# zjzijielu/graphsage-simple

Measured on AMD Instinct MI355X. Metric: node-embeddings/sec (2-hop forward), higher is better.
Workload: dtype f32

## Files before the change

### experiments/l2_placement_trace.py

```python
import collections
import csv
import glob
import sys

import numpy as np

f = sorted(glob.glob(sys.argv[1] + "/**/*_kernel_trace.csv", recursive=True))[-1]
edge = int(sys.argv[2]) if len(sys.argv) > 2 else 40


def kind(n):
    if "sample_kernel" in n:
        return "So" if "true, true>" in n else "Si"
    if "layer1_phase_kernel" in n:
        return "G"
    if "layer_tile16" in n or "layer_fused" in n:
        return "L"
    return None


rows = []
for r in csv.DictReader(open(f)):
    k = kind(r["Kernel_Name"])
    if k:
        rows.append((int(r["Start_Timestamp"]), int(r["End_Timestamp"]), k, r.get("Queue_Id", "?")))
rows.sort()
phases = [[rows[0]]]
last = rows[0][1]
for r in rows[1:]:
    if r[0] - last > 300_000:
        phases.append([])
    phases[-1].append(r)
    last = max(last, r[1])
cands = [ph for ph in phases if 100 * 4 <= len(ph) <= 1000 * 4]
big = [ph for ph in phases if len(ph) >= 100 * 4]
p = cands[-1] if cands else big[-1] if big else max(phases, key=len)
print("phases (kernels): " + " ".join(str(len(ph)) for ph in phases if len(ph) >= 50))
by = collections.defaultdict(list)
queues = collections.defaultdict(collections.Counter)
for s, e, k, q in p:
    by[k].append((s, e))
    queues[k][q] += 1
n = min(220, min(len(v) for v in by.values()))
S = {k: np.array(v[-n:], dtype=np.float64) / 1e3 for k, v in by.items()}
assert all((S["L"][:, 0] > S["G"][:, 0]).tolist()) and all((S["G"][:, 0] > S["Si"][:, 0]).tolist()), "kernel kinds do not line up by batch"
lo, hi = edge, n - edge


def stat(x):
    x = np.asarray(x)
    return "avg %5.1f med %5.1f p10 %5.1f p90 %5.1f" % (x.mean(), np.median(x), np.percentile(x, 10), np.percentile(x, 90))


print(f"analysed phase: {n} batches, statistics over batches {lo} .. {hi - 1}")
print("period %.2f us" % ((S["L"][hi - 1, 1] - S["L"][lo, 1]) / (hi - 1 - lo)))
for k in ("So", "Si", "G", "L"):
    print(f"  {k:2s} duration            {stat(S[k][lo:hi, 1] - S[k][lo:hi, 0])}")
print(f"  L(b) start - G(b) end    {stat(S['L'][lo:hi, 0] - S['G'][lo:hi, 1])}")
print(f"  L(b) start - G(b+1) start{stat(S['L'][lo:hi, 0] - S['G'][lo + 1:hi + 1, 0])}")
print(f"  L(b) end - G(b+1) start  {stat(S['L'][lo:hi, 1] - S['G'][lo + 1:hi + 1, 0])}")
print(f"  G(b+1) start - G(b) end  {stat(S['G'][lo + 1:hi + 1, 0] - S['G'][lo:hi, 1])}")
print(f"  G(b) start - Si(b) end   {stat(S['G'][lo:hi, 0] - S['Si'][lo:hi, 1])}")
print(f"  G(b) and G(b+1) together {stat(np.maximum(0.0, S['G'][lo:hi, 1] - S['G'][lo + 1:hi + 1, 0]))}")
print(f"  G end-to-end period      {stat(np.diff(S['G'][lo:hi + 1, 1]))}")
print("  queues used (whole phase): " + "  ".join(f"{k}: " + ", ".join(f"queue {q} x{c}" for q, c in sorted(queues[k].items())) for k in ("So", "Si", "G", "L")))
t0 = S["G"][lo, 0]
print("  timeline of four batches (us from G(b0) start):")
for b in range(lo, lo + 4):
    print("   b=%d " % b + "  ".join(f"{k} {S[k][b, 0] - t0:7.1f}->{S[k][b, 1] - t0:7.1f}" for k in ("So", "Si", "G", "L")))

depth = int(sys.argv[3]) if len(sys.argv) > 3 else 4
ev = sorted((s, e, k, q, i) for k in ("So", "Si", "G", "L") for i, ((s, e), q) in enumerate(zip(by[k][-n:], [r[3] for r in p if r[2] == k][-n:])))
prev_in_queue, last_of_queue = {}, {}
for s, e, k, q, i in ev:
    prev_in_queue[(k, i)] = last_of_queue.get(q)
    last_of_queue[q] = (k, i, e / 1e3)
Q = {(k, i): q for s, e, k, q, i in ev}
producer = {"Si": "So", "G": "Si", "L": "G"}
binding = {k: collections.Counter() for k in ("So", "Si", "G", "L")}
slack = {k: collections.defaultdict(list) for k in ("So", "Si", "G", "L")}
bound_by = {}
for k in ("So", "Si", "G", "L"):
    for b in range(lo, hi):
        start = S[k][b, 0]
        cons = {}
        pq = prev_in_queue[(k, b)]
        if pq:
            cons["queue:%s(b%+d)" % (pq[0], pq[1] - b)] = pq[2]
        if k in producer:
            cons["producer:%s(b)" % producer[k]] = S[producer[k]][b, 1]
        if k == "So" and b - depth >= 0:
            cons["release:L(b-%d)" % depth] = S["L"][b - depth, 1]
        name, t = max(cons.items(), key=lambda kv: kv[1])
        binding[k][name] += 1
        bound_by[(k, b)] = name
        slack[k][name].append(start - t)
print(f"last constraint met before each kernel start (batches {lo} .. {hi - 1}; depth {depth}): count, then start - constraint in us")
# ... 25 lines not shown
```

### graphsage-simple_amd/csrc/sage_api.hip

```cpp
#include <stdarg.h>
#include <string.h>

#include <stdlib.h>

#include <atomic>

#include "sage_internal.h"

static thread_local char g_err[512] = "";

void sage_set_error(const char* fmt, ...) {
    va_list ap;
    va_start(ap, fmt);
    vsnprintf(g_err, sizeof(g_err), fmt, ap);
    va_end(ap);
}

extern "C" int sage_abi_version(void) { return SAGE_ABI_VERSION; }
extern "C" const char* sage_last_error(void) { return g_err; }
extern "C" const char* sage_build_arch(void) { return "gfx950"; }

static int env_int(const char* name, int dflt, int lo, int hi) {
    const char* v = getenv(name);
    if (!v || !*v) return dflt;
    const long x = strtol(v, nullptr, 10);
    return (int)(x < lo ? lo : x > hi ? hi : x);
}

#ifndef SAGE_LAYER1_FUSED_DEFAULT
#define SAGE_LAYER1_FUSED_DEFAULT 1
#endif

const sage_tunables_t& sage_tunables() {
    static const sage_tunables_t t = [] {
        sage_tunables_t x;
        x.gather_blocks_per_cu = env_int("SAGE_G_PER_CU", 6, 1, 8);
        { const int sl = env_int("SAGE_G_SLICE_LANES", 0, 0, 64); x.gather_slice_lanes = (sl == 8 || sl == 16 || sl == 32 || sl == 64) ? sl : 0; }
        x.gather_rows_in_flight = env_int("SAGE_G_ROWS", 1, 1, 4);
        x.gather_trip = env_int("SAGE_G_TRIP", 16, 8, 16) >= 16 ? 16 : 8;
        x.gather_variant = env_int("SAGE_G_VARIANT", 1, 0, 2);
        x.gather_variant_sliced = env_int("SAGE_G_VARIANT_SM", getenv("SAGE_G_VARIANT") ? x.gather_variant : 2, 0, 2);
        x.dense_blocks = env_int("SAGE_DENSE_BLOCKS", 224, 32, 512);
        x.bwd_blocks = env_int("SAGE_BWD_BLOCKS", 512, 16, 4096);
        x.bwd_direct_blocks = env_int("SAGE_BWD_DIRECT_BLOCKS", 256, 16, 1024);
        const int so = env_int("SAGE_SO_THREADS", 512, 256, 1024);
        x.outer_threads = so >= 1024 ? 1024 : so >= 512 ? 512 : 256;
        x.tile16_grid = env_int("SAGE_T16_GRID", 2 * kNumCU, 64, 1024);
        x.sample_fused = env_int("SAGE_SAMPLE_FUSED", 0, 0, 1);
        { const int tw = env_int("SAGE_T16_WAVES", 0, 0, 16); x.tile16_waves = tw == 0 ? 0 : tw >= 16 ? 16 : 8; }
        { const int ti = env_int("SAGE_T16_INFLIGHT", 0, 0, 13); x.tile16_inflight = ti == 0 ? 0 : ti >= 13 ? 13 : 7; }
        x.layer1_fused = env_int("SAGE_LAYER1_FUSED", SAGE_LAYER1_FUSED_DEFAULT, 0, 1);
        x.layer1_phase_per_cu = env_int("SAGE_L1P_PER_CU", 3, 1, 3);
        return x;
    }();
    return t;
}

__global__ void sage_fill_u32_kernel(uint32_t* __restrict__ p, uint32_t v, size_t n_words) {
    for (size_t i = (size_t)blockIdx.x * blockDim.x + threadIdx.x; i < n_words; i += (size_t)gridDim.x * blockDim.x) p[i] = v;
}
int sage_fill_u32(void* p, uint32_t v, size_t n_words, hipStream_t st) {
    if (n_words == 0) return SAGE_OK;
    const int blocks = (int)(n_words < 256 ? 1 : (n_words / 256 < 1024 ? n_words / 256 : 1024));
    hipLaunchKernelGGL(sage_fill_u32_kernel, dim3(blocks), dim3(256), 0, st, (uint32_t*)p, v, n_words);
    SAGE_CHECK_LAUNCH("sage_fill_u32_kernel");
    return SAGE_OK;
}
```

### graphsage-simple_amd/csrc/sage_gather_body.h

```cpp
#pragma once
#include "sage_internal.h"

namespace sage_gather_detail {

template <int SL>
__device__ __forceinline__ void gather_sliced_block(
    const float* __restrict__ table, int table_rows, int64_t ld, int dim,
    const int32_t* __restrict__ nbr, const int32_t* __restrict__ cnt, int k, int n, const int32_t* __restrict__ n_dev,
    const int32_t* __restrict__ slot_rows, const int32_t* __restrict__ self_row, const int32_t* __restrict__ any_nonempty,
    float* __restrict__ out, int64_t ldo, int n_off, int nslice, const int bid, const int nblk, const int64_t slice_stride = 0, const int act = SAGE_ACT_NONE) {
    using V = __attribute__((ext_vector_type(4))) float;
    constexpr int NPI = kWave / SL;
#ifdef SAGE_G_INFLIGHT
    constexpr int U = SAGE_G_INFLIGHT;
#else
    constexpr int U = 8 / NPI;
#endif
    int nn = n;
    if (n_dev) nn = min(*n_dev + n_off, n);
    const int lane = sage_lane();
    const int slice = (int)(bid % nslice);
    const int wave = (int)(((bid / nslice) * blockDim.x + threadIdx.x) >> 6);
    const int nwaves = (int)(((nblk / nslice) * blockDim.x) >> 6);
    const int grp = lane / SL, gl = lane % SL;
// ... 80 lines not shown
            if (self_row) s_cur[i] = self_row[r];
        }
    }
    while (r0 < nn) {
        const int rn0 = r0 + R * nwaves;
        int c_nxt[R], id_nxt[R], s_nxt[R];
#pragma unroll
        for (int i = 0; i < R; ++i) {
            const int r = rn0 + i * nwaves;
            c_nxt[i] = 0; id_nxt[i] = 0; s_nxt[i] = -1;
            if (r < nn) {
                c_nxt[i] = cnt[r];
                id_nxt[i] = (lane < k) ? nbr[(int64_t)r * k + lane] : 0;
                if (self_row) s_nxt[i] = self_row[r];
            }
        }
        int cc[R], ss[R], ids[R];
        bool extra[R];
        V t[R][U];
#pragma unroll
        for (int i = 0; i < R; ++i) {
            cc[i] = min(__builtin_amdgcn_readfirstlane(c_cur[i]), kWave);
            int s = s_cur[i];
            if (slot_rows && s >= 0) s = slot_rows[s];
            ss[i] = __builtin_amdgcn_readfirstlane(s);
            int myid = (lane < cc[i]) ? id_cur[i] : 0;
            if (slot_rows) myid = slot_rows[max(myid, 0)];
            extra[i] = ss[i] >= 0;
            if (extra[i] && __any(lane < cc[i] && myid == ss[i])) extra[i] = false;
            ids[i] = min(max(myid, 0), last_row);
#pragma unroll
            for (int u = 0; u < U; ++u) {
                const int j = u * NPI + grp;
                const int id = __shfl(ids[i], min(j, max(cc[i] - 1, 0)), kWave);
                if (ok && j < cc[i]) t[i][u] = *reinterpret_cast<const V*>(tcol + (int64_t)id * ld);
                else t[i][u] = V{0.f, 0.f, 0.f, 0.f};
            }
        }
#pragma unroll
        for (int i = 0; i < R; ++i) {
            const int r = r0 + i * nwaves;
            if (r >= nn) continue;
            const int c = cc[i];
            V acc = {0.f, 0.f, 0.f, 0.f};
#pragma unroll
            for (int u = 0; u < U; ++u) acc += t[i][u];
            for (int j0 = NPI * U; j0 < c; j0 += NPI * U) {
                V w[U];
#pragma unroll
                for (int u = 0; u < U; ++u) {
                    const int j = j0 + u * NPI + grp;
                    const int id = __shfl(ids[i], min(j, c - 1), kWave);
                    if (ok && j < c) w[u] = *reinterpret_cast<const V*>(tcol + (int64_t)id * ld);
                    else w[u] = V{0.f, 0.f, 0.f, 0.f};
                }
#pragma unroll
                for (int u = 0; u < U; ++u) acc += w[u];
            }
            if (extra[i] && ok && grp == 0) acc += *reinterpret_cast<const V*>(tcol + (int64_t)min(ss[i], last_row) * ld);
#pragma unroll
            for (int m = SL; m < kWave; m <<= 1) {
                acc[0] += __shfl_xor(acc[0], m, kWave);
                acc[1] += __shfl_xor(acc[1], m, kWave);
                acc[2] += __shfl_xor(acc[2], m, kWave);
                acc[3] += __shfl_xor(acc[3], m, kWave);
            }
            if (grp == 0 && ok) {
                const int ceff = c + (extra[i] ? 1 : 0);
                V res;
                if (ceff > 0) res = acc * (1.0f / (float)ceff);
                else { const float fill = nan_rule ? __builtin_nanf("") : 0.f; res = V{fill, fill, fill, fill}; }
                if (act != SAGE_ACT_NONE) { res[0] = sage_activate(res[0], act); res[1] = sage_activate(res[1], act); res[2] = sage_activate(res[2], act); res[3] = sage_activate(res[3], act); }
            sage_store_stream<SAGE_AGG_STORE>(reinterpret_cast<V*>(out + (int64_t)r * ldo + c0), res);
            }
        }
        r0 = rn0;
#pragma unroll
        for (int i = 0; i < R; ++i) { c_cur[i] = c_nxt[i]; id_cur[i] = id_nxt[i]; s_cur[i] = s_nxt[i]; }
    }
}

using gather_v4 = __attribute__((ext_vector_type(4))) float;
template <int TRIP, bool SLOT>
__device__ __forceinline__ gather_v4 gather_rows_unit_sum(const float* __restrict__ tcol, const int64_t ld, const int32_t* __restrict__ myn,
                                                          const int c, const int k, const int s, const int last_row,
                                                          const int32_t* __restrict__ slot_rows, bool& extra) {
    using V = gather_v4;
    V acc = {0.f, 0.f, 0.f, 0.f};
    for (int j0 = 0; j0 < k; j0 += TRIP) {
        int id[TRIP];
#pragma unroll
        for (int u = 0; u < TRIP; ++u) id[u] = myn[min(min(j0 + u, c - 1), k - 1) < 0 ? 0 : min(min(j0 + u, c - 1), k - 1)];
        V t[TRIP];
#pragma unroll
        for (int u = 0; u < TRIP; ++u) {
            int x = id[u];
            if (SLOT) x = slot_rows[max(x, 0)];
            extra = extra && !(j0 + u < c && x == s);
            x = min(max(x, 0), last_row);
            t[u] = *reinterpret_cast<const V*>(tcol + (int64_t)x * ld);
        }
#pragma unroll
        for (int u = 0; u < TRIP; ++u) {
            acc[0] += (j0 + u < c) ? t[u][0] : 0.f; acc[1] += (j0 + u < c) ? t[u][1] : 0.f;
            acc[2] += (j0 + u < c) ? t[u][2] : 0.f; acc[3] += (j0 + u < c) ? t[u][3] : 0.f;
        }
    }
    if (extra) {
        const V sv = *reinterpret_cast<const V*>(tcol + (int64_t)min(s, last_row) * ld);
        acc += sv;
    }
    return acc;
}
__device__ __forceinline__ gather_v4 gather_rows_unit_mean(const gather_v4 acc, const int c, const bool extra, const bool nan_rule) {
    const int ceff = c + (extra ? 1 : 0);
    if (ceff > 0) return acc * (1.0f / (float)ceff);
    const float fill = nan_rule ? __builtin_nanf("") : 0.f;
    return gather_v4{fill, fill, fill, fill};
}

template <int SL, int TRIP, bool SLOT>
__device__ __forceinline__ void gather_sliced_block_rows(
    const float* __restrict__ table, int table_rows, int64_t ld, int dim,
    const int32_t* __restrict__ nbr, const int32_t* __restrict__ cnt, int k, int n, const int32_t* __restrict__ n_dev,
    const int32_t* __restrict__ slot_rows, const int32_t* __restrict__ self_row, const int32_t* __restrict__ any_nonempty,
    float* __restrict__ out, int64_t ldo, int n_off, int nslice, const int bid, const int nblk, const int64_t slice_stride = 0, const int act = SAGE_ACT_NONE) {
    using V = __attribute__((ext_vector_type(4))) float;
    constexpr int NG = kWave / SL;
    int nn = n;
    if (n_dev) nn = min(*n_dev + n_off, n);
    const int lane = sage_lane();
    const int slice = (int)(bid % nslice);
    const int wave = (int)(((bid / nslice) * blockDim.x + threadIdx.x) >> 6);
    const int nwaves = (int)(((nblk / nslice) * blockDim.x) >> 6);
    const int grp = lane / SL, gl = lane % SL;
    const int c0 = min(slice * SL * 4 + gl * 4, dim - 4);
    const bool ok = slice * SL * 4 + gl * 4 < dim;
    const bool nan_rule = any_nonempty ? (*any_nonempty != 0) : false;
    const int last_row = table_rows - 1;
    const float* __restrict__ tcol = table + (slice_stride ? (int64_t)slice * slice_stride + min(gl * 4, SL * 4 - 4) : (int64_t)c0);
    const int nblocks_rows = (nn + NG - 1) / NG;
    for (int rb = wave; rb < nblocks_rows; rb += nwaves) {
        const int r = rb * NG + grp;
        const bool valid = r < nn;
        const int rq = valid ? r : nn - 1;
        const int c = min(cnt[rq], k);
        int s = -1;
        if (self_row) {
            s = self_row[rq];
            if (SLOT && s >= 0) s = slot_rows[s];
        }
        bool extra = s >= 0;
        const int32_t* __restrict__ myn = nbr + (int64_t)rq * k;
        const V acc = gather_rows_unit_sum<TRIP, SLOT>(tcol, ld, myn, c, k, s, last_row, slot_rows, extra);
        if (valid && ok) {
            V res = gather_rows_unit_mean(acc, c, extra, nan_rule);
            if (act != SAGE_ACT_NONE) { res[0] = sage_activate(res[0], act); res[1] = sage_activate(res[1], act); res[2] = sage_activate(res[2], act); res[3] = sage_activate(res[3], act); }
            sage_store_stream<SAGE_AGG_STORE>(reinterpret_cast<V*>(out + (int64_t)r * ldo + c0), res);
        }
    }
}

}
```

### graphsage-simple_amd/csrc/sage_internal.h

```cpp
#pragma once
#include "sage_common.h"

struct sage_resolve_t {
    const int32_t* slots; int32_t* rows_out; int32_t n_slots;
    const int32_t* self_slots; int32_t* self_rows_out; int32_t n_self;
    const int32_t* hash_rows; int32_t* hash_keys;
};
struct sage_slot_resolve_t {
    int32_t* wipe_keys;
    int32_t* rows_out;
    int32_t* self_rows_out;
};
struct sage_finish_t {
    int32_t* counters;
    int32_t* cursor;
};
struct sage_rows_t {
    const float* table; int64_t table_rows; int64_t ld; int32_t dim;
    int64_t slice_stride = 0;
};
struct sage_lists_t {
    const int32_t* nbr = nullptr;
    const int32_t* cnt = nullptr;
    int32_t k = 0;
// ... 35 lines not shown
    const sage_model_t* queue_model = nullptr;
    int nodes_from_batch = 0;
    int32_t* nodes_copy = nullptr;
    const int32_t* seed_map = nullptr;
    const sage_resolve_t* resolve = nullptr;
};
int sage_launch_sample(const sage_sample_t& s, hipStream_t st, sage_launch_events_t* ev = nullptr);
int sage_launch_sample_wide(const sage_sample_t& s, hipStream_t st);
int sage_check_frontier(const sage_frontier_t* f, int64_t inserts);

struct sage_sample_fused_t {
    const sage_model_t* m; const int32_t* seeds; int32_t batch; uint64_t seed; int queued = 0;
    int32_t* nbr2; int32_t* cnt2; int32_t* any2 = nullptr;
    const sage_frontier_t* frontier; int32_t frontier_row_off = 0; int32_t insert_self = 0; int32_t* nbr_slot; int32_t* self_slot = nullptr;
    int32_t* nodes_copy = nullptr;
    int32_t* nbr1; int32_t* cnt1; int32_t* any1 = nullptr; int32_t seed_rows = 0;
};
int sage_launch_sample_fused(const sage_sample_fused_t& s, hipStream_t st);

int sage_launch_gather_mean(const sage_rows_t& src, const sage_lists_t& l, float* out, int64_t ldo, int32_t act, hipStream_t st,
                            sage_launch_events_t* ev = nullptr);
bool sage_layer_dense_supported(int32_t dim, int32_t out_dim);
bool sage_gather_is_sliced(int32_t dim, int64_t ld, int64_t ldo, const float* table, const float* out, int32_t n, int32_t k);

int sage_launch_linear_act(const sage_rows_t& agg, const sage_lists_t& rows, const sage_self_t& self, const sage_contract_t& c,
                           sage_finish_t fin, hipStream_t st);

enum sage_layer_company_t {
    SAGE_BESIDE_ANYTHING = 0,
    SAGE_BESIDE_ONE_WAVE_LAYER1 = 1,
    SAGE_BESIDE_LAYER1_AND_INNER_SAMPLER = 2,
};
int sage_launch_layer_fused(const sage_rows_t& src, const sage_lists_t& l, const sage_self_t& self, const sage_contract_t& c,
                            const sage_slot_resolve_t* resolve, sage_finish_t fin, hipStream_t st, sage_launch_events_t* ev = nullptr,
                            sage_layer_company_t company = SAGE_BESIDE_ANYTHING);
bool sage_layer_fused_supported(int32_t dim, int32_t out_dim, int32_t concat);
int sage_launch_layer_dense(const sage_rows_t& agg, const sage_lists_t& rows, const sage_self_t& self, const sage_contract_t& c,
                            sage_finish_t fin, hipStream_t st, sage_launch_events_t* ev = nullptr);

bool sage_layer1_phase_supported(int32_t d0, int32_t h1, int32_t k);
int sage_launch_layer1_phase(const sage_rows_t& src, const sage_lists_t& l, const sage_contract_t& c, hipStream_t st,
                             sage_launch_events_t* ev = nullptr);

struct sage_head_t {
    const float* emb; int64_t lde; int32_t dim;
    const float* w_cls; int64_t ldw; int32_t num_classes;
    const int64_t* labels = nullptr; int32_t n; float scale = 1.f;
    float* scores = nullptr; int64_t lds = 0; int32_t* pred = nullptr;
    float* grad_emb = nullptr; int64_t ldg = 0;
    float* part_w = nullptr; float* part_loss = nullptr;
    float* grad_w = nullptr; int64_t ldgw = 0; float* loss = nullptr;
};
int sage_launch_xent_head(const sage_head_t& h, hipStream_t st);

#define SAGE_STAGE_SAMPLE_OUTER 1
#define SAGE_STAGE_SAMPLE_INNER 2
#define SAGE_STAGE_GATHER1      4
#define SAGE_STAGE_CONTRACT1    8
#define SAGE_STAGE_LAYER2       16
#define SAGE_STAGE_ALL          31
int sage_forward2_launch_stages(const sage_model_t* m, void* workspace, size_t workspace_bytes, const int32_t* seeds, int32_t batch,
                                uint64_t seed, float* out, int64_t ldo, int32_t stages, hipStream_t stream, void* tail_event = nullptr,
                                void* const* gather_events = nullptr, bool inner_with_layer1 = false);

bool sage_forward2_contract1_is_empty(const sage_model_t* m, int32_t batch);
bool sage_forward2_sampler_is_fused(const sage_model_t* m);

struct sage_tunables_t {
    int gather_blocks_per_cu;
    int gather_slice_lanes;
    int gather_rows_in_flight;
    int gather_trip;
    int gather_variant;
    int gather_variant_sliced;
    int dense_blocks;
    int bwd_blocks;
    int bwd_direct_blocks;
    int outer_threads;
    int tile16_grid;
    int sample_fused;
    int tile16_waves;
    int tile16_inflight;
    int layer1_fused;
    int layer1_phase_per_cu;
};
int sage_fill_u32(void* p, uint32_t v, size_t n_words, hipStream_t st);
const sage_tunables_t& sage_tunables();

#ifndef SAGE_SPLIT_MIN_DIM
#define SAGE_SPLIT_MIN_DIM 64
#endif

#ifdef __HIPCC__
struct sage_finish_regs { int32_t c[7]; int32_t cur; };

__device__ inline void sage_finish_begin(const sage_finish_t& fin, sage_finish_regs& r) {
    if (!fin.counters || threadIdx.x != 0) return;
#pragma unroll
    for (int i = 0; i < 7; ++i) r.c[i] = fin.counters[i];
    r.cur = fin.cursor ? *fin.cursor : 0;
}

__device__ inline void sage_finish_block(const sage_finish_t& fin, int total_blocks, const sage_finish_regs& r) {
    if (!fin.counters) return;
    __syncthreads();
    if (threadIdx.x == 0) {
        if (__hip_atomic_fetch_add(&fin.counters[7], 1, __ATOMIC_RELAXED, __HIP_MEMORY_SCOPE_AGENT) == total_blocks - 1) {
#pragma unroll
            for (int i = 0; i < 7; ++i) {
                fin.counters[8 + i] = r.c[i];
                fin.counters[i] = 0;
            }
            fin.counters[7] = 0;
            if (fin.cursor) *fin.cursor = r.cur + 1;
        }
    }
}

__device__ inline void sage_finish_block(const sage_finish_t& fin, int total_blocks) {
    sage_finish_regs r;
    sage_finish_begin(fin, r);
    sage_finish_block(fin, total_blocks, r);
}
#endif
```

### graphsage-simple_amd/csrc/sage_layer1_phase.hip

```cpp
#include "sage_gather_body.h"
#include "sage_split_bf16.h"

namespace {

using namespace sage_split_detail;
using sage_gather_detail::gather_rows_unit_mean;
using sage_gather_detail::gather_rows_unit_sum;
using sage_gather_detail::gather_v4;

struct PhaseArgs {
    const float* table; int table_rows; int64_t slice_stride;
    const int32_t* nbr; const int32_t* cnt; int k;
    int n; const int32_t* n_dev; int n_off;
    const int32_t* self_row; const int32_t* any_nonempty;
    const float* W; int64_t ldw; const uint4* wsplit; int out_dim; int act;
    float* out; int64_t ldo;
};

constexpr int kTileRows = 32;
constexpr int kSliceFloats = 32;
constexpr int kMaxK = SAGE_MAX_FANOUT;

__device__ inline float exact_mean(const PhaseArgs& a, const int32_t* ids, int c, int s, bool extra, bool nan_rule, int kk) {
    const int last_row = a.table_rows - 1;
    const float* col = a.table + (int64_t)(kk / kSliceFloats) * a.slice_stride + (kk % kSliceFloats);
    float sum = 0.f;
    for (int j = 0; j < c; ++j) sum += col[(int64_t)min(max(ids[j], 0), last_row) * kSliceFloats];
    if (extra) sum += col[(int64_t)min(s, last_row) * kSliceFloats];
    const int ceff = c + (extra ? 1 : 0);
    if (ceff > 0) return sum * (1.0f / (float)ceff);
    return nan_rule ? __builtin_nanf("") : 0.f;
}

template <int NSLICE>
__global__ __launch_bounds__(256, 3) void layer1_phase_kernel(const PhaseArgs a) {
    constexpr int M = kTileRows, SL = 8, TRIP = 16;
    constexpr int LDB = kSliceFloats + 8;
    constexpr int PL = M * LDB;
    constexpr int PLD = 128 + 4;
    constexpr int STEPS = NSLICE;
    __shared__ __attribute__((aligned(16))) __bf16 planes[2 * 3 * PL];
    __shared__ __attribute__((aligned(16))) float outp[M * PLD];
    __shared__ int32_t ids[M * kMaxK];
    __shared__ int32_t cnts[M], selfs[M];
    __shared__ int rowflag[M];
    __shared__ int tileflag;

    const int tid = threadIdx.x, lane = tid & 63, wave = tid >> 6;
    int nn = a.n;
    if (a.n_dev) nn = min(*a.n_dev + a.n_off, a.n);
    const int ntiles = (nn + M - 1) / M;
    const bool nan_rule = a.any_nonempty ? (*a.any_nonempty != 0) : false;
    const int last_row = a.table_rows - 1;
    const int grp = lane / SL, gl = lane % SL;
    const int lr = wave * (kWave / SL) + grp;
    const int i32 = lane & 31, h = lane >> 5;
    const int n0 = wave * 32;
    const bool mfma_wave = n0 < a.out_dim;
    const int k = a.k;
    const bool w_huge = a.wsplit[(size_t)8 * STEPS * 3 * 64].x != 0;

    for (int tile = (int)blockIdx.x; tile < ntiles; tile += (int)gridDim.x) {
        __syncthreads();
        for (int i = tid; i < M * k; i += 256) {
            const int rq = min(tile * M + i / k, nn - 1);
            ids[i] = a.nbr[(int64_t)rq * k + i % k];
        }
        if (tid < M) {
            const int rq = min(tile * M + tid, nn - 1);
            cnts[tid] = min(a.cnt[rq], k);
            selfs[tid] = a.self_row ? a.self_row[rq] : -1;
            rowflag[tid] = 0;
        }
        if (tid == 0) tileflag = w_huge ? 1 : 0;
        __syncthreads();
        const bool valid = tile * M + lr < nn;
        const int c = cnts[lr], s = selfs[lr];
        const int32_t* myn = ids + lr * k;

        f32x16 acc[2];
#pragma unroll
        for (int e = 0; e < 16; ++e) { acc[0][e] = 0.f; acc[1][e] = 0.f; }
#pragma unroll
        for (int kg = 0; kg < 2; ++kg) {
#pragma unroll 1
            for (int q = 0; q < NSLICE / 2; ++q) {
                const int p = kg * (NSLICE / 2) + q;
                const float* tcol = a.table + (int64_t)p * a.slice_stride + gl * 4;
                bool extra = s >= 0;
                const gather_v4 sum = gather_rows_unit_sum<TRIP, false>(tcol, kSliceFloats, myn, c, k, s, last_row, nullptr, extra);
                bf16x8 bw[2][3];
                {
                    const uint4* wp = a.wsplit + ((size_t)(kg * 4 + __builtin_amdgcn_readfirstlane(wave)) * STEPS + 2 * q) * 3 * 64;
#pragma unroll
                    for (int j = 0; j < 2; ++j)
#pragma unroll
                        for (int pl = 0; pl < 3; ++pl) bw[j][pl] = __builtin_bit_cast(bf16x8, wp[(j * 3 + pl) * 64 + lane]);
                }
                gather_v4 res = gather_rows_unit_mean(sum, c, extra, nan_rule);
                if (!valid) res = gather_v4{0.f, 0.f, 0.f, 0.f};
                if (huge4(res)) { rowflag[lr] = 1; tileflag = 1; }
                __bf16* buf = planes + (p & 1) * 3 * PL;
                {
                    bf16x4 hi, mid, lo;
                    split3(res, hi, mid, lo);
                    __bf16* dst = buf + lr * LDB + gl * 4;
                    *reinterpret_cast<bf16x4*>(dst) = hi;
                    *reinterpret_cast<bf16x4*>(dst + PL) = mid;
                    *reinterpret_cast<bf16x4*>(dst + 2 * PL) = lo;
                }
                lds_barrier();
                if (mfma_wave) {
                    const __bf16* abase = buf + i32 * LDB + 8 * h;
#pragma unroll
                    for (int j = 0; j < 2; ++j) {
                        const bf16x8 ah = *reinterpret_cast<const bf16x8*>(abase + 16 * j);
                        const bf16x8 am = *reinterpret_cast<const bf16x8*>(abase + PL + 16 * j);
                        const bf16x8 al = *reinterpret_cast<const bf16x8*>(abase + 2 * PL + 16 * j);
                        acc[kg] = mfma_bf16x3_step(ah, am, al, bw[j], acc[kg]);
                    }
                }
            }
        }
        if (mfma_wave) {
            float* mine = outp + n0 + i32;
#pragma unroll
            for (int reg = 0; reg < 16; ++reg) mine[((reg & 3) + 8 * (reg >> 2) + 4 * h) * PLD] = acc[0][reg] + acc[1][reg];
        }
        lds_barrier();
        const bool any_bad = tileflag != 0;
#pragma unroll
        for (int it = 0; it < M * 32 / 256; ++it) {
            const int idx = it * 256 + tid;
            const int row = idx >> 5, col = (idx & 31) * 4;
            const int g = tile * M + row;
            if (g < nn && col < a.out_dim && !(any_bad && (w_huge || rowflag[row] != 0))) {
                const f32x4 pv = *reinterpret_cast<const f32x4*>(outp + row * PLD + col);
                f32x4 v;
#pragma unroll
                for (int e = 0; e < 4; ++e) v[e] = sage_activate(pv[e], a.act);
                sage_store_stream<SAGE_H1_STORE>(reinterpret_cast<f32x4*>(a.out + (int64_t)g * a.ldo + col), v);
            }
        }
        if (any_bad) {
            const int d0 = NSLICE * kSliceFloats;
            for (int idx = tid; idx < M * a.out_dim; idx += 256) {
                const int row = idx / a.out_dim, col = idx % a.out_dim;
                const int g = tile * M + row;
                if (g >= nn || !(w_huge || rowflag[row] != 0)) continue;
                const int32_t* rid = ids + row * k;
                const int rc = cnts[row], rs = selfs[row];
                bool rextra = rs >= 0;
                for (int j = 0; j < rc; ++j) rextra = rextra && rid[j] != rs;
                const float* wrow = a.W + (int64_t)col * a.ldw;
                float dot = 0.f;
                for (int kk = 0; kk < d0; ++kk) dot = fmaf(exact_mean(a, rid, rc, rs, rextra, nan_rule, kk), wrow[kk], dot);
                a.out[(int64_t)g * a.ldo + col] = sage_activate(dot, a.act);
            }
        }
    }
}

template <int NSLICE>
int launch_phase(const PhaseArgs& a, hipStream_t st, sage_launch_events_t* ev) {
    const int per_cu = sage_tunables().layer1_phase_per_cu;
    const int grid = min((sage_cdiv(a.n, kTileRows) + 7) / 8 * 8, kNumCU * per_cu);
    sage_launch(layer1_phase_kernel<NSLICE>, dim3(grid), dim3(256), 0, st, ev, a);
    SAGE_CHECK_LAUNCH("layer1_phase_kernel");
    return SAGE_OK;
}

}

bool sage_layer1_phase_supported(int32_t d0, int32_t h1, int32_t k) {
    return (d0 == 64 || d0 == 128 || d0 == 256) && h1 >= 32 && h1 <= 128 && h1 % 32 == 0 && k >= 1 && k <= kMaxK;
}

int sage_launch_layer1_phase(const sage_rows_t& src, const sage_lists_t& l, const sage_contract_t& c, hipStream_t st,
                             sage_launch_events_t* ev) {
    const int32_t d0 = src.dim;
    SAGE_REQUIRE(src.ld == kSliceFloats && src.slice_stride == src.table_rows * (int64_t)kSliceFloats,
                 "layer1_fused: the table must be slice-major with %d-float slices", kSliceFloats);
    if (!sage_layer1_phase_supported(d0, c.out_dim, l.k) || !c.weight_prepared || !sage_aligned(src.table, 16) || !sage_aligned(c.out, 16) ||
        !sage_aligned(c.weight_prepared, 16) || c.ldo % 4 != 0 || c.ldo < c.out_dim || c.ldw < d0) {
        sage_set_error("layer1_fused: unsupported shape d0=%d h1=%d k=%d (or unaligned arrays / no prepared weights)", d0, c.out_dim, l.k);
        return SAGE_EUNSUPPORTED;
    }
    if (l.n == 0) return SAGE_OK;
    const PhaseArgs a{src.table, (int)src.table_rows, src.slice_stride, l.nbr, l.cnt, l.k, l.n, l.n_dev, l.n_off, l.self_row, l.any_nonempty,
                      c.weight, c.ldw, (const uint4*)c.weight_prepared, c.out_dim, c.act, c.out, c.ldo};
    if (d0 == 64) return launch_phase<2>(a, st, ev);
    if (d0 == 128) return launch_phase<4>(a, st, ev);
    return launch_phase<8>(a, st, ev);
}

extern "C" int sage_layer1_fused_supported(int32_t d0, int32_t h1, int32_t k) { return sage_layer1_phase_supported(d0, h1, k) ? 1 : 0; }

extern "C" int sage_layer1_fused(const float* table_sliced, int64_t table_rows, int32_t d0, const int32_t* nbr, const int32_t* cnt,
                                 int32_t k, int32_t n, const int32_t* n_dev, const int32_t* self_row, const int32_t* any_nonempty,
                                 const float* weight, int64_t ldw, const void* weight_prepared, int32_t out_dim, int32_t act, float* out,
                                 int64_t ldo, sage_stream_t stream) {
    SAGE_REQUIRE(table_sliced && nbr && cnt && weight && weight_prepared && out, "layer1_fused: NULL array");
    SAGE_REQUIRE(n >= 0 && table_rows >= 1 && table_rows < (1ll << 31), "layer1_fused: n = %d, table_rows = %lld", n, (long long)table_rows);
    SAGE_REQUIRE(act >= 0 && act <= SAGE_ACT_NONE, "layer1_fused: bad activation");
    return sage_launch_layer1_phase({.table = table_sliced, .table_rows = table_rows, .ld = kSliceFloats, .dim = d0,
                                     .slice_stride = table_rows * (int64_t)kSliceFloats},
                                    {.nbr = nbr, .cnt = cnt, .k = k, .n = n, .n_dev = n_dev, .self_row = self_row, .any_nonempty = any_nonempty},
                                    {.weight = weight, .ldw = ldw, .weight_prepared = weight_prepared, .out_dim = out_dim, .act = act, .out = out,
                                     .ldo = ldo},
                                    (hipStream_t)stream);
}
```

Baseline: 80.82 million.

## Add two-tile layer-1 pair kernel that overlaps neighbour gathers with contraction

Adds a layer1_pair_kernel where each block processes two 32-row tiles at once. The neighbour-row gathers for one tile are issued in halves while the other tile's sums and MFMA contraction run, so memory latency is hidden by software pipelining with sched barriers. The kernel is specialised on self-row and long-fanout cases and is the default (SAGE_L1P_TILES=2), with occupancy reduced to 2 blocks per CU. The existing kernel is refactored into shared helpers. The costs are more registers and lower occupancy in exchange for more loads in flight per wave.

```diff
diff --git a/experiments/l2_placement_trace.py b/experiments/l2_placement_trace.py
--- a/experiments/l2_placement_trace.py
+++ b/experiments/l2_placement_trace.py
@@ -12,7 +12,7 @@
 def kind(n):
     if "sample_kernel" in n:
         return "So" if "true, true>" in n else "Si"
-    if "layer1_phase_kernel" in n:
+    if "layer1_phase_kernel" in n or "layer1_pair_kernel" in n:
         return "G"
     if "layer_tile16" in n or "layer_fused" in n:
         return "L"
diff --git a/graphsage-simple_amd/csrc/sage_api.hip b/graphsage-simple_amd/csrc/sage_api.hip
--- a/graphsage-simple_amd/csrc/sage_api.hip
+++ b/graphsage-simple_amd/csrc/sage_api.hip
@@ -31,6 +31,10 @@
 #define SAGE_LAYER1_FUSED_DEFAULT 1
 #endif
 
+#ifndef SAGE_L1P_TILES_DEFAULT
+#define SAGE_L1P_TILES_DEFAULT 2
+#endif
+
 const sage_tunables_t& sage_tunables() {
     static const sage_tunables_t t = [] {
         sage_tunables_t x;
@@ -50,7 +54,8 @@
         { const int tw = env_int("SAGE_T16_WAVES", 0, 0, 16); x.tile16_waves = tw == 0 ? 0 : tw >= 16 ? 16 : 8; }
         { const int ti = env_int("SAGE_T16_INFLIGHT", 0, 0, 13); x.tile16_inflight = ti == 0 ? 0 : ti >= 13 ? 13 : 7; }
         x.layer1_fused = env_int("SAGE_LAYER1_FUSED", SAGE_LAYER1_FUSED_DEFAULT, 0, 1);
-        x.layer1_phase_per_cu = env_int("SAGE_L1P_PER_CU", 3, 1, 3);
+        x.layer1_phase_tiles = env_int("SAGE_L1P_TILES", SAGE_L1P_TILES_DEFAULT, 1, 2);
+        { const int most = x.layer1_phase_tiles == 2 ? 2 : 3; x.layer1_phase_per_cu = env_int("SAGE_L1P_PER_CU", most, 1, most); }
         return x;
     }();
     return t;
diff --git a/graphsage-simple_amd/csrc/sage_gather_body.h b/graphsage-simple_amd/csrc/sage_gather_body.h
--- a/graphsage-simple_amd/csrc/sage_gather_body.h
+++ b/graphsage-simple_amd/csrc/sage_gather_body.h
@@ -186,35 +186,53 @@
 
 using gather_v4 = __attribute__((ext_vector_type(4))) float;
 template <int TRIP, bool SLOT>
+__device__ __forceinline__ void gather_rows_unit_issue(const float* __restrict__ tcol, const int64_t ld, const int32_t* __restrict__ myn,
+                                                       const int j0, const int c, const int k, const int s, const int last_row,
+                                                       const int32_t* __restrict__ slot_rows, bool& extra, gather_v4 (&t)[TRIP]) {
+    int id[TRIP];
+#pragma unroll
+    for (int u = 0; u < TRIP; ++u) id[u] = myn[min(min(j0 + u, c - 1), k - 1) < 0 ? 0 : min(min(j0 + u, c - 1), k - 1)];
+#pragma unroll
+    for (int u = 0; u < TRIP; ++u) {
+        int x = id[u];
+        if (SLOT) x = slot_rows[max(x, 0)];
+        extra = extra && !(j0 + u < c && x == s);
+        x = min(max(x, 0), last_row);
+        t[u] = *reinterpret_cast<const gather_v4*>(tcol + (int64_t)x * ld);
+    }
+}
+template <int TRIP>
+__device__ __forceinline__ void gather_rows_unit_add(gather_v4& acc, const gather_v4 (&t)[TRIP], const int j0, const int c) {
+#pragma unroll
+    for (int u = 0; u < TRIP; ++u) {
+        acc[0] += (j0 + u < c) ? t[u][0] : 0.f; acc[1] += (j0 + u < c) ? t[u][1] : 0.f;
+        acc[2] += (j0 + u < c) ? t[u][2] : 0.f; acc[3] += (j0 + u < c) ? t[u][3] : 0.f;
+    }
+}
+template <int TRIP, bool SLOT>
 __device__ __forceinline__ gather_v4 gather_rows_unit_sum(const float* __restrict__ tcol, const int64_t ld, const int32_t* __restrict__ myn,
                                                           const int c, const int k, const int s, const int last_row,
                                                           const int32_t* __restrict__ slot_rows, bool& extra) {
     using V = gather_v4;
     V acc = {0.f, 0.f, 0.f, 0.f};
     for (int j0 = 0; j0 < k; j0 += TRIP) {
-        int id[TRIP];
-#pragma unroll
-        for (int u = 0; u < TRIP; ++u) id[u] = myn[min(min(j0 + u, c - 1), k - 1) < 0 ? 0 : min(min(j0 + u, c - 1), k - 1)];
         V t[TRIP];
-#pragma unroll
-        for (int u = 0; u < TRIP; ++u) {
-            int x = id[u];
-            if (SLOT) x = slot_rows[max(x, 0)];
-            extra = extra && !(j0 + u < c && x == s);
-            x = min(max(x, 0), last_row);
-            t[u] = *reinterpret_cast<const V*>(tcol + (int64_t)x * ld);
-        }
-#pragma unroll
-        for (int u = 0; u < TRIP; ++u) {
-            acc[0] += (j0 + u < c) ? t[u][0] : 0.f; acc[1] += (j0 + u < c) ? t[u][1] : 0.f;
-            acc[2] += (j0 + u < c) ? t[u][2] : 0.f; acc[3] += (j0 + u < c) ? t[u][3] : 0.f;
-        }
+        gather_rows_unit_issue<TRIP, SLOT>(tcol, ld, myn, j0, c, k, s, last_row, slot_rows, extra, t);
+        gather_rows_unit_add<TRIP>(acc, t, j0, c);
     }
     if (extra) {
         const V sv = *reinterpret_cast<const V*>(tcol + (int64_t)min(s, last_row) * ld);
         acc += sv;
     }
     return acc;
+}
+__device__ __forceinline__ float gather_rows_unit_scale(const int c, const bool extra) {
+    const int ceff = c + (extra ? 1 : 0);
+    return ceff > 0 ? 1.0f / (float)ceff : -1.0f;
+}
+__device__ __forceinline__ gather_v4 gather_rows_unit_mean(const gather_v4 acc, const float scale, const bool nan_rule) {
+    const float fill = nan_rule ? __builtin_nanf("") : 0.f;
+    return scale >= 0.f ? acc * scale : gather_v4{fill, fill, fill, fill};
 }
 __device__ __forceinline__ gather_v4 gather_rows_unit_mean(const gather_v4 acc, const int c, const bool extra, const bool nan_rule) {
     const int ceff = c + (extra ? 1 : 0);
diff --git a/graphsage-simple_amd/csrc/sage_internal.h b/graphsage-simple_amd/csrc/sage_internal.h
--- a/graphsage-simple_amd/csrc/sage_internal.h
+++ b/graphsage-simple_amd/csrc/sage_internal.h
@@ -141,6 +141,7 @@
     int tile16_waves;
     int tile16_inflight;
     int layer1_fused;
+    int layer1_phase_tiles;
     int layer1_phase_per_cu;
 };
 int sage_fill_u32(void* p, uint32_t v, size_t n_words, hipStream_t st);
diff --git a/graphsage-simple_amd/csrc/sage_layer1_phase.hip b/graphsage-simple_amd/csrc/sage_layer1_phase.hip
--- a/graphsage-simple_amd/csrc/sage_layer1_phase.hip
+++ b/graphsage-simple_amd/csrc/sage_layer1_phase.hip
@@ -4,7 +4,10 @@
 namespace {
 
 using namespace sage_split_detail;
+using sage_gather_detail::gather_rows_unit_add;
+using sage_gather_detail::gather_rows_unit_issue;
 using sage_gather_detail::gather_rows_unit_mean;
+using sage_gather_detail::gather_rows_unit_scale;
 using sage_gather_detail::gather_rows_unit_sum;
 using sage_gather_detail::gather_v4;
 
@@ -20,6 +23,9 @@
 constexpr int kTileRows = 32;
 constexpr int kSliceFloats = 32;
 constexpr int kMaxK = SAGE_MAX_FANOUT;
+constexpr int kOutLd = 128 + 4;
+constexpr int kPlaneLd = kSliceFloats + 8;
+constexpr int kPlane = kTileRows * kPlaneLd;
 
 __device__ inline float exact_mean(const PhaseArgs& a, const int32_t* ids, int c, int s, bool extra, bool nan_rule, int kk) {
     const int last_row = a.table_rows - 1;
@@ -32,12 +38,90 @@
     return nan_rule ? __builtin_nanf("") : 0.f;
 }
 
+template <int STEPS>
+__device__ __forceinline__ void load_w1_phase(const uint4* wsplit, const int kg, const int q, const int wave, const int lane, bf16x8 (&bw)[2][3]) {
+    const uint4* wp = wsplit + ((size_t)(kg * 4 + __builtin_amdgcn_readfirstlane(wave)) * STEPS + 2 * q) * 3 * 64;
+#pragma unroll
+    for (int j = 0; j < 2; ++j)
+#pragma unroll
+        for (int pl = 0; pl < 3; ++pl) bw[j][pl] = __builtin_bit_cast(bf16x8, wp[(j * 3 + pl) * 64 + lane]);
+}
+
+__device__ __forceinline__ f32x16 contract_slice(const gather_v4 res, __bf16* buf, const int lr, const int gl, const int lane, const bool mfma_wave,
+                                                 int* rowflag_lr, int* tileflag, const bf16x8 (&bw)[2][3], f32x16 acc) {
+    constexpr int LDB = kPlaneLd, PL = kPlane;
+    if (huge4(res)) { *rowflag_lr = 1; *tileflag = 1; }
+    {
+        bf16x4 hi, mid, lo;
+        split3(res, hi, mid, lo);
+        __bf16* dst = buf + lr * LDB + gl * 4;
+        *reinterpret_cast<bf16x4*>(dst) = hi;
+        *reinterpret_cast<bf16x4*>(dst + PL) = mid;
+        *reinterpret_cast<bf16x4*>(dst + 2 * PL) = lo;
+    }
+    lds_barrier();
+    if (mfma_wave) {
+        const __bf16* abase = buf + (lane & 31) * LDB + 8 * (lane >> 5);
+#pragma unroll
+        for (int j = 0; j < 2; ++j) {
+            const bf16x8 ah = *reinterpret_cast<const bf16x8*>(abase + 16 * j);
+            const bf16x8 am = *reinterpret_cast<const bf16x8*>(abase + PL + 16 * j);
+            const bf16x8 al = *reinterpret_cast<const bf16x8*>(abase + 2 * PL + 16 * j);
+            acc = mfma_bf16x3_step(ah, am, al, bw[j], acc);
+        }
+    }
+    return acc;
+}
+
+template <int NSLICE>
+__device__ __forceinline__ void tile_epilogue(const PhaseArgs& a, const int tile, const int nn, const f32x16 (&acc)[2], float* outp,
+                                              const int32_t* ids, const int32_t* cnts, const int32_t* selfs, const int* rowflag,
+                                              const int* tileflag, const bool w_huge, const bool nan_rule) {
+    constexpr int M = kTileRows, PLD = kOutLd;
+    const int tid = threadIdx.x, lane = tid & 63, wave = tid >> 6;
+    const int i32 = lane & 31, h = lane >> 5, n0 = wave * 32, k = a.k;
+    if (n0 < a.out_dim) {
+        float* mine = outp + n0 + i32;
+#pragma unroll
+        for (int reg = 0; reg < 16; ++reg) mine[((reg & 3) + 8 * (reg >> 2) + 4 * h) * PLD] = acc[0][reg] + acc[1][reg];
+    }
+    lds_barrier();
+    const bool any_bad = *tileflag != 0;
+#pragma unroll 1
+    for (int it = 0; it < M * 32 / 256; ++it) {
+        const int idx = it * 256 + tid;
+        const int row = idx >> 5, col = (idx & 31) * 4;
+        const int g = tile * M + row;
+        if (g < nn && col < a.out_dim && !(any_bad && (w_huge || rowflag[row] != 0))) {
+            const f32x4 pv = *reinterpret_cast<const f32x4*>(outp + row * PLD + col);
+            f32x4 v;
+#pragma unroll
+            for (int e = 0; e < 4; ++e) v[e] = sage_activate(pv[e], a.act);
+            sage_store_stream<SAGE_H1_STORE>(reinterpret_cast<f32x4*>(a.out + (int64_t)g * a.ldo + col), v);
+        }
+    }
+    if (any_bad) {
+        const int d0 = NSLICE * kSliceFloats;
+        for (int idx = tid; idx < M * a.out_dim; idx += 256) {
+            const int row = idx / a.out_dim, col = idx % a.out_dim;
+            const int g = tile * M + row;
+            if (g >= nn || !(w_huge || rowflag[row] != 0)) continue;
+            const int32_t* rid = ids + row * k;
+            const int rc = cnts[row], rs = selfs[row];
+            bool rextra = rs >= 0;
+            for (int j = 0; j < rc; ++j) rextra = rextra && rid[j] != rs;
+            const float* wrow = a.W + (int64_t)col * a.ldw;
+            float dot = 0.f;
+            for (int kk = 0; kk < d0; ++kk) dot = fmaf(exact_mean(a, rid, rc, rs, rextra, nan_rule, kk), wrow[kk], dot);
+            a.out[(int64_t)g * a.ldo + col] = sage_activate(dot, a.act);
+        }
+    }
+}
+
 template <int NSLICE>
 __global__ __launch_bounds__(256, 3) void layer1_phase_kernel(const PhaseArgs a) {
     constexpr int M = kTileRows, SL = 8, TRIP = 16;
-    constexpr int LDB = kSliceFloats + 8;
-    constexpr int PL = M * LDB;
-    constexpr int PLD = 128 + 4;
+    constexpr int PL = kPlane, PLD = kOutLd;
     constexpr int STEPS = NSLICE;
     __shared__ __attribute__((aligned(16))) __bf16 planes[2 * 3 * PL];
     __shared__ __attribute__((aligned(16))) float outp[M * PLD];
@@ -54,9 +138,7 @@
     const int last_row = a.table_rows - 1;
     const int grp = lane / SL, gl = lane % SL;
     const int lr = wave * (kWave / SL) + grp;
-    const int i32 = lane & 31, h = lane >> 5;
-    const int n0 = wave * 32;
-    const bool mfma_wave = n0 < a.out_dim;
+    const bool mfma_wave = wave * 32 < a.out_dim;
     const int k = a.k;
     const bool w_huge = a.wsplit[(size_t)8 * STEPS * 3 * 64].x != 0;
 
@@ -90,80 +172,158 @@
                 bool extra = s >= 0;
                 const gather_v4 sum = gather_rows_unit_sum<TRIP, false>(tcol, kSliceFloats, myn, c, k, s, last_row, nullptr, extra);
                 bf16x8 bw[2][3];
-                {
-                    const uint4* wp = a.wsplit + ((size_t)(kg * 4 + __builtin_amdgcn_readfirstlane(wave)) * STEPS + 2 * q) * 3 * 64;
-#pragma unroll
-                    for (int j = 0; j < 2; ++j)
-#pragma unroll
-                        for (int pl = 0; pl < 3; ++pl) bw[j][pl] = __builtin_bit_cast(bf16x8, wp[(j * 3 + pl) * 64 + lane]);
-                }
+                load_w1_phase<STEPS>(a.wsplit, kg, q, wave, lane, bw);
                 gather_v4 res = gather_rows_unit_mean(sum, c, extra, nan_rule);
                 if (!valid) res = gather_v4{0.f, 0.f, 0.f, 0.f};
-                if (huge4(res)) { rowflag[lr] = 1; tileflag = 1; }
-                __bf16* buf = planes + (p & 1) * 3 * PL;
-                {
-                    bf16x4 hi, mid, lo;
-                    split3(res, hi, mid, lo);
-                    __bf16* dst = buf + lr * LDB + gl * 4;
-                    *reinterpret_cast<bf16x4*>(dst) = hi;
-                    *reinterpret_cast<bf16x4*>(dst + PL) = mid;
-                    *reinterpret_cast<bf16x4*>(dst + 2 * PL) = lo;
-                }
-                lds_barrier();
-                if (mfma_wave) {
-                    const __bf16* abase = buf + i32 * LDB + 8 * h;
-#pragma unroll
-                    for (int j = 0; j < 2; ++j) {
-                        const bf16x8 ah = *reinterpret_cast<const bf16x8*>(abase + 16 * j);
-                        const bf16x8 am = *reinterpret_cast<const bf16x8*>(abase + PL + 16 * j);
-                        const bf16x8 al = *reinterpret_cast<const bf16x8*>(abase + 2 * PL + 16 * j);
-                        acc[kg] = mfma_bf16x3_step(ah, am, al, bw[j], acc[kg]);
-                    }
-                }
+                acc[kg] = contract_slice(res, planes + (p & 1) * 3 * kPlane, lr, gl, lane, mfma_wave, &rowflag[lr], &tileflag, bw, acc[kg]);
             }
         }
-        if (mfma_wave) {
-            float* mine = outp + n0 + i32;
-#pragma unroll
-            for (int reg = 0; reg < 16; ++reg) mine[((reg & 3) + 8 * (reg >> 2) + 4 * h) * PLD] = acc[0][reg] + acc[1][reg];
-        }
+        tile_epilogue<NSLICE>(a, tile, nn, acc, outp, ids, cnts, selfs, rowflag, &tileflag, w_huge, nan_rule);
+    }
+}
+
+template <int NSLICE, bool SELF, bool LONG>
+__global__ __launch_bounds__(256, 2) void layer1_pair_kernel(const PhaseArgs a) {
+    constexpr int M = kTileRows, SL = 8, HALF = 8;
+    constexpr int MORE = 4;
+    constexpr int PL = kPlane, PLD = kOutLd;
+    constexpr int STEPS = NSLICE;
+    __shared__ __attribute__((aligned(16))) __bf16 planes[2 * 3 * PL];
+    __shared__ __attribute__((aligned(16))) float outp[M * PLD];
+    __shared__ int32_t ids[2 * M * kMaxK];
+    __shared__ int32_t cnts[2 * M], selfs[2 * M];
+    __shared__ int rowflag[2 * M];
+    __shared__ int tileflag[2];
+
+    const int tid = threadIdx.x, lane = tid & 63, wave = tid >> 6;
+    int nn = a.n;
+    if (a.n_dev) nn = min(*a.n_dev + a.n_off, a.n);
+    const int npairs = (nn + 2 * M - 1) / (2 * M);
+    const bool nan_rule = a.any_nonempty ? (*a.any_nonempty != 0) : false;
+    const int last_row = a.table_rows - 1;
+    const int grp = lane / SL, gl = lane % SL;
+    const int lr = wave * (kWave / SL) + grp;
+    const bool mfma_wave = wave * 32 < a.out_dim;
+    const int k = a.k;
+    const bool w_huge = a.wsplit[(size_t)8 * STEPS * 3 * 64].x != 0;
+
+    for (int pair = (int)blockIdx.x; pair < npairs; pair += (int)gridDim.x) {
+        __syncthreads();
+        {
+            const int row = tid >> 2;
+            const int rq = min(pair * 2 * M + row, nn - 1);
+            for (int j = tid & 3; j < k; j += 4) ids[row * k + j] = a.nbr[(int64_t)rq * k + j];
+        }
+        if (tid < 2 * M) {
+            const int rq = min(pair * 2 * M + tid, nn - 1);
+            cnts[tid] = min(a.cnt[rq], k);
+            selfs[tid] = SELF ? a.self_row[rq] : -1;
+            rowflag[tid] = 0;
+        }
+        if (tid < 2) tileflag[tid] = w_huge ? 1 : 0;
+        __syncthreads();
+        bool valid[2], extra[2];
+        float scale[2];
+        int c[2], s[2];
+        const int32_t* myn[2];
+#pragma unroll
+        for (int t = 0; t < 2; ++t) {
+            valid[t] = pair * 2 * M + t * M + lr < nn;
+            c[t] = cnts[t * M + lr];
+            s[t] = selfs[t * M + lr];
+            myn[t] = ids + (t * M + lr) * k;
+            extra[t] = SELF && s[t] >= 0;
+            if (SELF)
+                for (int j = 0; j < c[t]; ++j) extra[t] = extra[t] && myn[t][j] != s[t];
+            scale[t] = gather_rows_unit_scale(c[t], extra[t]);
+        }
+        auto issue = [&](const int t, const int p, const int h, gather_v4 (&rows)[HALF], gather_v4& selfv) __attribute__((always_inline)) {
+            const float* tcol = a.table + (int64_t)p * a.slice_stride + gl * 4;
+            bool unused = false;
+            const int cnow = cnts[t * M + lr];
+            gather_rows_unit_issue<HALF, false>(tcol, kSliceFloats, myn[t], HALF * h, cnow, k, -1, last_row, nullptr, unused, rows);
+            if (SELF && h == 0) selfv = *reinterpret_cast<const gather_v4*>(tcol + (int64_t)min(max(selfs[t * M + lr], 0), last_row) * kSliceFloats);
+        };
+        auto finish = [&](const int t, const int p, gather_v4 sum, const gather_v4 selfv) __attribute__((always_inline)) {
+            const float* tcol = a.table + (int64_t)p * a.slice_stride + gl * 4;
+            const int cnow = cnts[t * M + lr];
+            for (int j0 = 2 * HALF; LONG && j0 < k; j0 += MORE) {
+                gather_v4 more[MORE];
+                bool unused = false;
+                gather_rows_unit_issue<MORE, false>(tcol, kSliceFloats, myn[t], j0, cnow, k, -1, last_row, nullptr, unused, more);
+                gather_rows_unit_add<MORE>(sum, more, j0, cnow);
+            }
+            if (SELF) {
+                const gather_v4 with = sum + selfv;
+                if (extra[t]) sum = with;
+            }
+            gather_v4 res = gather_rows_unit_mean(sum, scale[t], nan_rule);
+            if (!valid[t]) res = gather_v4{0.f, 0.f, 0.f, 0.f};
+            return res;
+        };
+
+        f32x16 acc[2][2];
+#pragma unroll
+        for (int e = 0; e < 16; ++e) { acc[0][0][e] = 0.f; acc[0][1][e] = 0.f; acc[1][0][e] = 0.f; acc[1][1][e] = 0.f; }
+        gather_v4 rows_a[2][HALF], self_a = {0.f, 0.f, 0.f, 0.f};
+        issue(0, 0, 0, rows_a[0], self_a);
+        issue(0, 0, 1, rows_a[1], self_a);
+        auto phase = [&](const int kg, const int q, const bool last) __attribute__((always_inline)) {
+            const int p = kg * (NSLICE / 2) + q;
+            gather_v4 rows_b[2][HALF], self_b = {0.f, 0.f, 0.f, 0.f};
+            gather_v4 sum = {0.f, 0.f, 0.f, 0.f};
+            bf16x8 bw[2][3];
+            load_w1_phase<STEPS>(a.wsplit, kg, q, wave, lane, bw);
+            __builtin_amdgcn_sched_barrier(0);
+            gather_rows_unit_add<HALF>(sum, rows_a[0], 0, cnts[lr]);
+            __builtin_amdgcn_sched_barrier(0);
+            issue(1, p, 0, rows_b[0], self_b);
+            __builtin_amdgcn_sched_barrier(0);
+            gather_rows_unit_add<HALF>(sum, rows_a[1], HALF, cnts[lr]);
+            __builtin_amdgcn_sched_barrier(0);
+            issue(1, p, 1, rows_b[1], self_b);
+            __builtin_amdgcn_sched_barrier(0);
+            const gather_v4 res_a = finish(0, p, sum, self_a);
+            acc[0][kg] = contract_slice(res_a, planes, lr, gl, lane, mfma_wave, &rowflag[lr], &tileflag[0], bw, acc[0][kg]);
+            sum = gather_v4{0.f, 0.f, 0.f, 0.f};
+            __builtin_amdgcn_sched_barrier(0);
+            gather_rows_unit_add<HALF>(sum, rows_b[0], 0, cnts[M + lr]);
+            __builtin_amdgcn_sched_barrier(0);
+            if (!last) issue(0, p + 1, 0, rows_a[0], self_a);
+            __builtin_amdgcn_sched_barrier(0);
+            gather_rows_unit_add<HALF>(sum, rows_b[1], HALF, cnts[M + lr]);
+            __builtin_amdgcn_sched_barrier(0);
+            if (!last) issue(0, p + 1, 1, rows_a[1], self_a);
+            __builtin_amdgcn_sched_barrier(0);
+            const gather_v4 res_b = finish(1, p, sum, self_b);
+            acc[1][kg] = contract_slice(res_b, planes + 3 * PL, lr, gl, lane, mfma_wave, &rowflag[M + lr], &tileflag[1], bw, acc[1][kg]);
+        };
+#pragma unroll 1
+        for (int q = 0; q < NSLICE / 2; ++q) phase(0, q, false);
+#pragma unroll 1
+        for (int q = 0; q < NSLICE / 2 - 1; ++q) phase(1, q, false);
+        phase(1, NSLICE / 2 - 1, true);
+
+        tile_epilogue<NSLICE>(a, 2 * pair, nn, acc[0], outp, ids, cnts, selfs, rowflag, &tileflag[0], w_huge, nan_rule);
         lds_barrier();
-        const bool any_bad = tileflag != 0;
-#pragma unroll
-        for (int it = 0; it < M * 32 / 256; ++it) {
-            const int idx = it * 256 + tid;
-            const int row = idx >> 5, col = (idx & 31) * 4;
-            const int g = tile * M + row;
-            if (g < nn && col < a.out_dim && !(any_bad && (w_huge || rowflag[row] != 0))) {
-                const f32x4 pv = *reinterpret_cast<const f32x4*>(outp + row * PLD + col);
-                f32x4 v;
-#pragma unroll
-                for (int e = 0; e < 4; ++e) v[e] = sage_activate(pv[e], a.act);
-                sage_store_stream<SAGE_H1_STORE>(reinterpret_cast<f32x4*>(a.out + (int64_t)g * a.ldo + col), v);
-            }
-        }
-        if (any_bad) {
-            const int d0 = NSLICE * kSliceFloats;
-            for (int idx = tid; idx < M * a.out_dim; idx += 256) {
-                const int row = idx / a.out_dim, col = idx % a.out_dim;
-                const int g = tile * M + row;
-                if (g >= nn || !(w_huge || rowflag[row] != 0)) continue;
-                const int32_t* rid = ids + row * k;
-                const int rc = cnts[row], rs = selfs[row];
-                bool rextra = rs >= 0;
-                for (int j = 0; j < rc; ++j) rextra = rextra && rid[j] != rs;
-                const float* wrow = a.W + (int64_t)col * a.ldw;
-                float dot = 0.f;
-                for (int kk = 0; kk < d0; ++kk) dot = fmaf(exact_mean(a, rid, rc, rs, rextra, nan_rule, kk), wrow[kk], dot);
-                a.out[(int64_t)g * a.ldo + col] = sage_activate(dot, a.act);
-            }
-        }
+        tile_epilogue<NSLICE>(a, 2 * pair + 1, nn, acc[1], outp, ids + M * k, cnts + M, selfs + M, rowflag + M, &tileflag[1], w_huge, nan_rule);
     }
 }
 
 template <int NSLICE>
 int launch_phase(const PhaseArgs& a, hipStream_t st, sage_launch_events_t* ev) {
-    const int per_cu = sage_tunables().layer1_phase_per_cu;
+    const sage_tunables_t& tn = sage_tunables();
+    const int per_cu = tn.layer1_phase_per_cu;
+    if (tn.layer1_phase_tiles == 2) {
+        const int grid = min((sage_cdiv(a.n, 2 * kTileRows) + 7) / 8 * 8, kNumCU * per_cu);
+        const bool self = a.self_row != nullptr, lng = a.k > 16;
+        if (self && lng) sage_launch(layer1_pair_kernel<NSLICE, true, true>, dim3(grid), dim3(256), 0, st, ev, a);
+        else if (self) sage_launch(layer1_pair_kernel<NSLICE, true, false>, dim3(grid), dim3(256), 0, st, ev, a);
+        else if (lng) sage_launch(layer1_pair_kernel<NSLICE, false, true>, dim3(grid), dim3(256), 0, st, ev, a);
+        else sage_launch(layer1_pair_kernel<NSLICE, false, false>, dim3(grid), dim3(256), 0, st, ev, a);
+        SAGE_CHECK_LAUNCH("layer1_pair_kernel");
+        return SAGE_OK;
+    }
     const int grid = min((sage_cdiv(a.n, kTileRows) + 7) / 8 * 8, kNumCU * per_cu);
     sage_launch(layer1_phase_kernel<NSLICE>, dim3(grid), dim3(256), 0, st, ev, a);
     SAGE_CHECK_LAUNCH("layer1_phase_kernel");
```

Result: faster. 83.43 million, median of 6 (+3.2%).
